# Excalibur-SLE/spmv

Measured on AMD Instinct MI355X. Metric: fp64 CG iters/sec (SpMV effective GB/s vs HBM roofline), higher is better.
Workload: dtype f64

## Files before the change

spmv_amd/csrc/hip/csr_plan.h:

```cpp
#pragma once

#include "common.h"

#include <chrono>
#include <cstdio>

constexpr int kRows = kBlock;

typedef double f64x2 __attribute__((ext_vector_type(2)));
typedef float f32x4 __attribute__((ext_vector_type(4)));
typedef int i32x2 __attribute__((ext_vector_type(2)));
typedef int i32x4 __attribute__((ext_vector_type(4)));

template <typename T>
struct VecOf;
template <>
struct VecOf<double> {
  static constexpr int V = 2;
  using val_t = f64x2;
  using col_t = i32x2;
};
template <>
struct VecOf<float> {
  static constexpr int V = 4;
// ... 81 lines not shown
constexpr int kLxRec = 36;
constexpr int kLxCap = 1344;
constexpr int kLxGap = 16;
constexpr int kLxwPiece = 128;
constexpr int kLxwMaxPieces = 16;
constexpr int kLxwPieces0 = 4;
constexpr int kLxwNpMask = 0xff;
constexpr int kLxwOwnShift = 8;
constexpr int kLxwOwnMask = 0xfffff;
constexpr int kLxwCodedBit = 30;
constexpr int kLxwDict0 = kLxwPieces0 + kLxwMaxPieces;
constexpr int kLxwDictSize = 16;
constexpr int kLxwRec = 28;
__host__ __device__ constexpr int64_t lx_code_bytes(int64_t nnz)
{
  return (((nnz + 1) >> 1) + 16 + 15) & ~(int64_t)15;
}
__host__ __device__ constexpr int64_t lx32_len(int64_t nnz)
{
  return (nnz + 3) & ~(int64_t)3;
}
constexpr int kLxwAlign = 4;
constexpr int kLxwRingValRounds = 2;
constexpr int kLxwRingVcap = kLxwRingValRounds * 1024;
constexpr int kLxwRingCodeMax = 4096;
__host__ __device__ constexpr int lx_ring_code_bytes(int cnt)
{
  return (cnt + 31 + 7) / 8 * 4 + 8;
}
__host__ __device__ constexpr bool lx_ring_fits(int cnt)
{
  return cnt > 0 && cnt + 3 <= kLxwRingVcap
         && lx_ring_code_bytes(cnt) <= kLxwRingCodeMax;
}
constexpr int kXwMaxWin = 8;
constexpr int kXwFirst0 = kLxwPieces0 + kLxwMaxPieces;
constexpr int kXwDelta0 = kXwFirst0 + kXwMaxWin;
constexpr int kXwRec = 36;

constexpr int kLatMaxOff = 8;
constexpr int kLatRec = 12;
constexpr int kWdiaMaxOff = 32;

struct PlanTrace {
  bool on;
  std::chrono::steady_clock::time_point t0;
  const char* who;
  explicit PlanTrace(const char* w)
      : on(getenv("SPMV_PLAN_TRACE") != nullptr), t0(std::chrono::steady_clock::now()),
        who(w)
  {
  }
  void mark(const char* what) const
  {
    if (!on)
      return;
    (void)hipDeviceSynchronize();
    fprintf(stderr, "%s %-14s %9.3f ms\n", who, what,
            std::chrono::duration<double, std::milli>(std::chrono::steady_clock::now()
                                                      - t0)
                .count());
  }
};

template <typename T>
static inline bool aligned16(const T* p)
// ... 136 lines not shown
  int sj_xcd_group = 8;
  struct SpmvTranspose* tr = nullptr;
  void* mv_scratch = nullptr;
  size_t mv_bytes = 0;
  int mv_form = 0;
  int mv_native = 1;
  int32_t* row_list = nullptr;
  int rowlist_exact = 0;
  int32_t num_listed = 0;
  int nt_store = 0;
  int plan_us = 0;
  int plan_mem_us = 0;
  int values_changed_us = 0;
  const int32_t* rowptr0 = nullptr;
  const int32_t* colind0 = nullptr;
  int released = 0;
  int no_new_forms = 0;
  bool structure_baked() const
  {
    return row_list || lx_lidx || lat_tab || slat_mask || t_ptr || lxw_rec
           || xw_rec || wdia_val || sj_lenperm;
  }
  uint16_t* lx_lidx = nullptr;
  int32_t* lx_tab = nullptr;
  int lx = 0;
  int lx_chunks = 2;
  int lx_staged = 0;
  int lx_blocks = 0;
  int32_t* lxw_rec = nullptr;
  int lxw = 0;
  int lxw_max_cnt = 0;
  int lxw_max_pieces = 0;
  int lxw_blocks_per_cu = 0;
  uint8_t* lx_code = nullptr;
  int lx4 = 0;
  int lx4_blocks = 0;
  int lx4_lut = 1;
  int lx_ring_blocks = 0;
  int lx_ring = 1;
  float* lx_val32 = nullptr;
  const void* lx32_values0 = nullptr;
  int lx_v32 = 0;
  int32_t* xw_rec = nullptr;
  int xw = 0;
  int xw_staged = 0;
  int xw_max_cnt = 0, xw_max_pieces = 0;
  struct XwProbe* xw_probe = nullptr;
  int32_t* lat_tab = nullptr;
  uint8_t* lat_mask = nullptr;
  int lat = 0;
  int lat_blocks = 0;
  int lat_blocks_per_cu = 4;
  int lat_xcd_group = 0;
  int lat_chain = 1;

  int lattice_d1 = 0, lattice_d2 = 0;

  int32_t* zw_table = nullptr;
  int zw_slots = 0;
  int zw_grid = 0;
  int zw_segments = 0;
  int64_t zw_d2 = 0;
  int zwalk = 0;

  RowBlockOrder row_block_order(int nrb) const
  {
    RowBlockOrder o;
    o.table = nullptr;
    o.num_slots = 0;
    o.xcd_group = xcd_group;
    o.num_row_blocks = nrb;
// ... 168 lines not shown
```

spmv_amd/csrc/hip/spmv_csr_forms.hip:

```cpp
#include "csr_plan.h"

#include <hipcub/hipcub.hpp>

#include <algorithm>
#include <chrono>
#include <cstring>
#include <new>
#include <utility>
#include <vector>

#include "plan_scratch.h"

namespace
{

template <int ITEMS>
__global__ __launch_bounds__(kBlock) void lx_build_kernel(
    int32_t num_rows, int32_t num_cols, const int32_t* __restrict__ rowptr,
    const int32_t* __restrict__ colind, uint16_t* __restrict__ lidx,
    int32_t* __restrict__ tab, int num_row_blocks, int end_bit, int align,
    int pad, int cap, int32_t* __restrict__ wrec, int32_t* __restrict__ stat,
    int xw)
{
  using Sort = hipcub::BlockRadixSort<int32_t, kBlock, ITEMS, int32_t>;
// ... 174 lines not shown
      }
      s_rank[kLx4Words] = n;
    }
    __syncthreads();
    if (s_rank[kLx4Words] > kLxwDictSize)
      continue;
    for (int w = t; w < kLx4Words; w += kBlock) {
      uint32_t m = s_bits[w];
      int k = s_rank[w];
      while (m) {
        const int b = __ffs(m) - 1;
        m &= m - 1;
        s_dict[k++] = w * 32 + b + kLx4Dmin;
      }
    }
    for (int32_t j = lo; j < hi; ++j) {
      const int b = (int)lidx[j] - t - kLx4Dmin;
      const uint32_t c
          = (uint32_t)(s_rank[b >> 5] + __popc(s_bits[b >> 5] & ((1u << (b & 31)) - 1u)));
      const int q = j - a0;
      atomicOr(&s_pack[q >> 3], c << ((q & 7) * 4));
    }
    __syncthreads();
    for (int w = t; w < nwords; w += kBlock) {
      const bool whole = (w > 0 || a0 == a) && (int64_t)a0 + 8 * (w + 1) <= (int64_t)a + cnt;
      uint32_t* dst = code + ((int64_t)a0 >> 3) + w;
      if (whole)
        *dst = s_pack[w];
      else if (s_pack[w])
        atomicOr(dst, s_pack[w]);
    }
    if (t < kLxwDictSize / 2)
      wr[kLxwDict0 + t] = (s_dict[2 * t] & 0xffff) | (s_dict[2 * t + 1] << 16);
    if (t == 0) {
      wr[3] |= 1 << kLxwCodedBit;
      ++coded;
      ring += lx_ring_fits(cnt) ? 1 : 0;
    }
  }
  if (t == 0 && coded)
    atomicAdd(&stat[0], coded);
  if (t == 0 && ring)
    atomicAdd(&stat[1], ring);
}

struct NonEmptyRow {
  const int32_t* rowptr;
  __device__ bool operator()(int i) const { return rowptr[i + 1] > rowptr[i]; }
};

}

void xw_probe_free(spmv_hip_csr_plan* pl)
{
  if (!pl->xw_probe)
    return;
  for (auto& e : pl->xw_probe->ev)
    for (hipEvent_t& h : e)
      if (h) {
        (void)hipEventDestroy(h);
        h = nullptr;
      }
  delete pl->xw_probe;
  pl->xw_probe = nullptr;
}

void xw_probe_drop_events(XwProbe* pb)
{
  for (auto& e : pb->ev)
    for (hipEvent_t& h : e)
      if (h) {
        (void)hipEventDestroy(h);
        h = nullptr;
      }
}

// ... 37 lines not shown
  hipStream_t st = pl->ctx->stream;
  const int n = pl->num_rows;
  const size_t cap = (size_t)(pl->nnz < n ? pl->nnz : n);
  PlanScratch<int32_t> d_count;
  PlanScratch<void> tmp;
  SPMV_CHECK_HIP(spmv_plan_malloc(&pl->row_list, sizeof(int32_t) * (cap ? cap : 1)));
  hipError_t e = d_count.alloc(1);
  hipcub::CountingInputIterator<int32_t> first(0);
  NonEmptyRow pred{rowptr};
  if (e == hipSuccess)
    e = plan_cub(tmp, [&](void* t, size_t& tb) {
      return hipcub::DeviceSelect::If(t, tb, first, pl->row_list, d_count.get(), n,
                                      pred, st);
    });
  int32_t count = 0;
  if (e == hipSuccess)
    e = plan_fetch(&count, d_count.get(), 1, st);
  tmp.reset();
  d_count.reset();
  if (e != hipSuccess) {
    plan_drop(pl->row_list);
    return static_cast<int>(e);
  }
  pl->num_listed = count;
  return SPMV_HIP_OK;
}

void spmv_free_lx(spmv_hip_csr_plan* pl)
{
  plan_drop(pl->lx_lidx);
  plan_drop(pl->lx_tab);
  plan_drop(pl->lxw_rec);
  plan_drop(pl->lx_code);
  pl->lx = pl->lx_staged = pl->lx_blocks = 0;
  pl->lxw = pl->lxw_max_cnt = pl->lxw_max_pieces = 0;
  pl->lx4 = pl->lx4_blocks = pl->lx_ring_blocks = 0;
  spmv_lx32_free(pl);
}

static int build_lx_codes(spmv_hip_csr_plan* pl, const int32_t* rowptr, int nrb,
                          hipStream_t st)
{
  const size_t bytes = (size_t)lx_code_bytes(pl->nnz);
  PlanScratch<int32_t> d_stat;
  hipError_t e = spmv_plan_malloc(&pl->lx_code, bytes);
  if (e == hipSuccess)
    e = d_stat.alloc(2);
  if (e == hipSuccess)
    e = hipMemsetAsync(pl->lx_code, 0, bytes, st);
  if (e == hipSuccess)
    e = hipMemsetAsync(d_stat.get(), 0, 2 * sizeof(int32_t), st);
  int32_t h_stat[2] = {0, 0};
  if (e == hipSuccess) {
    int grid = pl->ctx->num_cus * 8;
    grid = grid > nrb ? nrb : grid;
    hipLaunchKernelGGL(lx4_encode_kernel, dim3(grid), dim3(kBlock), 0, st,
                       pl->num_rows, rowptr, pl->lx_lidx, pl->lxw_rec,
                       reinterpret_cast<uint32_t*>(pl->lx_code), nrb, d_stat.get());
    e = hipGetLastError();
  }
  if (e == hipSuccess)
    e = plan_fetch(h_stat, d_stat.get(), 2, st);
  d_stat.reset();
  const int32_t coded = h_stat[0];
  if (e != hipSuccess || coded == 0) {
    (void)hipGetLastError();
    plan_drop(pl->lx_code);
    pl->lx4 = pl->lx4_blocks = pl->lx_ring_blocks = 0;
    return e == hipSuccess || e == hipErrorOutOfMemory ? SPMV_HIP_OK
                                                       : static_cast<int>(e);
// ... 321 lines not shown
  PlanScratch<int32_t> d_count;
  PlanScratch<void> tmp;
  int32_t staged = 0;
  if (e == hipSuccess)
    e = d_count.alloc(1);
  hipcub::CountingInputIterator<int32_t> block_ids(0);
  hipcub::TransformInputIterator<int32_t, IsStagedRecord,
                                 hipcub::CountingInputIterator<int32_t>>
      flags(block_ids, IsStagedRecord{pl->lx_tab});
  if (e == hipSuccess)
    e = plan_cub(tmp, [&](void* t, size_t& tb) {
      return hipcub::DeviceReduce::Sum(t, tb, flags, d_count.get(), nrb, st);
    });
  if (e == hipSuccess)
    e = plan_fetch(&staged, d_count.get(), 1, st);
  tmp.reset();
  d_count.reset();
  d_stat.reset();
  if (e != hipSuccess) {
    spmv_free_lx(pl);
    return static_cast<int>(e);
  }
  pl->lx_blocks = nrb;
  pl->lx_staged = staged;
  pl->lxw_max_cnt = h_stat[0];
  pl->lxw_max_pieces = h_stat[1];
  if ((int64_t)staged * 2 < nrb) {
    spmv_free_lx(pl);
    pl->lx_blocks = nrb;
    return SPMV_HIP_OK;
  }
  pl->lx = 1;
  pl->lxw = pl->lxw_rec != nullptr;
  if (pl->lxw_rec && pl->ctx->lx_codes) {
    const int rc = build_lx_codes(pl, rowptr, nrb, st);
    if (rc != SPMV_HIP_OK)
      return rc;
  }
  pl->xcd_group = pl->nontemporal ? 16 : 0;
  {
    const int64_t d2 = spmv_plane_distance(pl, rowptr, colind);
    if (d2 > 0) {
      pl->lattice_d1 = 0;
      pl->lattice_d2 = (int)d2;
      const int rc = spmv_zwalk_order_build(pl, pl->lattice_d2,
                                            spmv_walk_grid(pl), 0, false);
      if (rc != SPMV_HIP_OK)
        return rc;
    }
  }
  return SPMV_HIP_OK;
}

int spmv_walk_grid(const spmv_hip_csr_plan* pl)
{
  if (pl->sdia && pl->sdia_val)
    return spmv_sdia_grid(pl);
  if (pl->symmetric)
    return spmv_slat_grid(pl);
  if (pl->lat_tab)
    return spmv_lat_grid(pl);
  if (pl->lxw && pl->lxw_rec)
    return spmv_lxw_grid(pl, 8);
  return (pl->xw && pl->xw_rec) ? spmv_xw_grid(pl, 8) : spmv_rowblock_grid(pl);
}

// ... 145 lines not shown
```

spmv_amd/csrc/hip/spmv_csr_plan.hip:

```cpp
#include "csr_plan.h"

#include <hipcub/hipcub.hpp>

#include <algorithm>
#include <chrono>
#include <cstring>
#include <new>
#include <utility>
#include <vector>

#include "plan_scratch.h"

thread_local int64_t spmv_plan_mem_ns = 0;

namespace
{
struct MemClock {
  spmv_hip_csr_plan* pl;
  int64_t t0;
  explicit MemClock(spmv_hip_csr_plan* p = nullptr) : pl(p), t0(spmv_plan_mem_ns) {}
  ~MemClock()
  {
    if (pl)
      pl->plan_mem_us += (int)((spmv_plan_mem_ns - t0) / 1000);
// ... 469 lines not shown
    SPMV_REQUIRE(value >= 0 && value <= 4096 && value % 256 == 0);
    plan->sym_window = value;
  } else if (!strcmp(key, "sym_rows")) {
    SPMV_REQUIRE(value == 512 || value == 1024 || value == 2048);
    plan->sym_rows = value;
  } else if (!strcmp(key, "blocks_per_cu")) {
    SPMV_REQUIRE(value >= 1 && value <= kBlocksPerCU);
    plan->blocks_per_cu = value;
    if (plan->zw_table && !plan->lat_tab && !plan->symmetric
        && !plan->sdia_val)
      return spmv_zwalk_order_build(plan, plan->zw_d2, spmv_walk_grid(plan), 0,
                                    true);
  } else if (!strcmp(key, "lx")) {
    SPMV_REQUIRE(value == 0 || plan->lx_lidx);
    plan->lx = value != 0;
  } else if (!strcmp(key, "lxw")) {
    SPMV_REQUIRE(value == 0 || plan->lxw_rec);
    plan->lxw = value != 0;
    if (plan->zw_table && plan->lx_lidx && !plan->lat_tab)
      return spmv_zwalk_order_build(plan, plan->zw_d2, spmv_walk_grid(plan), 0,
                                    true);
  } else if (!strcmp(key, "lx4")) {
    SPMV_REQUIRE(value == 0 || value == 1);
    SPMV_REQUIRE(value == 0 || plan->lx_code);
    plan->lx4 = value;
  } else if (!strcmp(key, "lx_v32")) {
    SPMV_REQUIRE(value == 0 || value == 1);
    SPMV_REQUIRE(value == 0 || plan->lx_val32);
    plan->lx_v32 = value;
  } else if (!strcmp(key, "lx_ring")) {
    SPMV_REQUIRE(value == 0 || value == 1);
    SPMV_REQUIRE(value == 0 || spmv_lxw_ring_ok(plan, true));
    plan->lx_ring = value ? 2 : 0;
  } else if (!strcmp(key, "lx4_lut")) {
    SPMV_REQUIRE(value == 1 || value == 2);
    plan->lx4_lut = value;
  } else if (!strcmp(key, "xw")) {
    SPMV_REQUIRE(value == 0 || plan->xw_rec);
    plan->xw = value != 0;
    if (plan->xw_probe && value) {
      plan->xw_probe->decided = 1;
      plan->xw_probe->use_xw = 1;
    }
    if (plan->zw_table && plan->xw_rec && !plan->lat_tab && !plan->lx_lidx)
      return spmv_zwalk_order_build(plan, plan->zw_d2, spmv_walk_grid(plan), 0,
                                    true);
  } else if (!strcmp(key, "xw_probe")) {
    SPMV_REQUIRE((value == 0 || value == 1) && plan->xw_rec);
    if (!plan->xw_probe)
      plan->xw_probe = new (std::nothrow) XwProbe;
    SPMV_REQUIRE(plan->xw_probe);
    xw_probe_drop_events(plan->xw_probe);
    *plan->xw_probe = XwProbe();
    plan->xw_probe->decided = value ? 0 : 1;
  } else if (!strcmp(key, "lxw_blocks_per_cu")) {
    SPMV_REQUIRE(value >= 0 && value <= kBlocksPerCU);
    plan->lxw_blocks_per_cu = value;
    if (plan->zw_table && !plan->lat_tab
        && ((plan->lxw_rec && plan->lxw) || (plan->xw_rec && plan->xw)))
      return spmv_zwalk_order_build(plan, plan->zw_d2, spmv_walk_grid(plan), 0,
                                    true);
  } else if (!strcmp(key, "lx_chunks")) {
    SPMV_REQUIRE(value == 1 || value == 2);
    plan->lx_chunks = value;
  } else if (!strcmp(key, "nt_store")) {
    plan->nt_store = value != 0;
// ... 221 lines not shown
  else if (!strcmp(key, "xw_pick"))
    *value = !(plan->xw && plan->xw_rec) ? 0
             : !plan->xw_probe           ? 1
             : plan->xw_probe->decided   ? plan->xw_probe->use_xw
                                         : -1;
  else if (!strcmp(key, "xw_probe_xw_us"))
    *value = plan->xw_probe ? (int)plan->xw_probe->us_xw : 0;
  else if (!strcmp(key, "xw_probe_gather_us"))
    *value = plan->xw_probe ? (int)plan->xw_probe->us_gather : 0;
  else if (!strcmp(key, "plan_us"))
    *value = plan->plan_us;
  else if (!strcmp(key, "plan_mem_us"))
    *value = plan->plan_mem_us;
  else if (!strcmp(key, "values_changed_us"))
    *value = plan->values_changed_us;
  else if (!strcmp(key, "mv_form"))
    *value = plan->mv_form;
  else if (!strcmp(key, "mv_native"))
    *value = plan->mv_native;
  else if (!strcmp(key, "mv_kib"))
    *value = (int)((plan->mv_bytes + 1023) / 1024);
  else if (!strcmp(key, "plan_kib")) {
    const int64_t n = plan->num_rows, nnz = plan->nnz;
    const int64_t nrb = (n + kRows - 1) / kRows;
    int64_t b = 0;
    if (plan->row_list)
      b += 4 * (int64_t)plan->num_listed;
    if (plan->lx_lidx)
      b += 2 * (nnz + 8) + 4 * nrb * kLxRec;
    if (plan->lxw_rec)
      b += 4 * nrb * kLxwRec;
    if (plan->lx_code)
      b += lx_code_bytes(nnz);
    if (plan->lx_val32)
      b += 4 * lx32_len(nnz);
    if (plan->xw_rec)
      b += 4 * nrb * kXwRec;
    if (plan->lat_tab)
      b += 48 * nrb + n;
    if (plan->slat_mask)
      b += n;
    const int64_t narr
        = plan->sdia_general == 2 ? 2 * plan->sdia_nd + 1 : plan->sdia_nd + 1;
    if (plan->sdia_val)
      b += narr * plan->sdia_len * plan->sdia_elem + n;
    if (plan->sdia32_val && !plan->sdia_const)
      b += narr * plan->sdia_len * 4 + n;
    if (plan->wdia_val)
      b += (int64_t)plan->wdia_narr * plan->wdia_len * plan->wdia_elem + 4 * n;
    if (plan->wdia32_val && !plan->wdia_const)
      b += (int64_t)plan->wdia_narr * plan->wdia_len * 4;
    if (plan->sj_lenperm)
      b += 4 * ((n + 63) / 64 * 64) + 8 * (int64_t)plan->sj_nblk
           + 4 * (int64_t)plan->sj_nblk * plan->sj_stride
           + (plan->sj_wide_alloc ? 4 : 2) * plan->sj_units * plan->sj_unit
           + 4 * (int64_t)plan->sj_nlong + 4 * ((n + 63) / 64 + 1)
           + 4 * plan->sj_lt_entries + 16 * (int64_t)plan->sj_lt_nsg
           + 2 * plan->sj_lt_codes_n + 8 * (int64_t)plan->sj_nlong;
    if (plan->sj_val)
      b += (int64_t)plan->sj_elem * plan->sj_units * plan->sj_unit;
    if (plan->sj_val32)
      b += 4 * plan->sj_units * plan->sj_unit;
    if (plan->sjt && plan->sjt->sj_lenperm) {
      const spmv_hip_csr_plan* c = plan->sjt;
      b += 4 * (n + 1) + (plan->sjv_map ? 4 * c->nnz : 0);
      if (plan->sj_long_rows)
// ... 50 lines not shown
    *value = plan->zwalk && plan->zw_table ? 1 : 0;
  else if (!strcmp(key, "zwalk_segments"))
    *value = plan->zw_table ? plan->zw_segments : 0;
  else if (!strcmp(key, "zwalk_grid"))
    *value = plan->zw_table ? plan->zw_grid : 0;
  else if (!strcmp(key, "lattice_d1"))
    *value = plan->lattice_d1;
  else if (!strcmp(key, "lattice_d2"))
    *value = plan->lattice_d2;
  else if (!strcmp(key, "lat"))
    *value = plan->lat;
  else if (!strcmp(key, "lat_chain"))
    *value = plan->lat_chain;
  else if (!strcmp(key, "lat_blocks"))
    *value = plan->lat_blocks;
  else if (!strcmp(key, "lx"))
    *value = plan->lx;
  else if (!strcmp(key, "lxw"))
    *value = plan->lxw && plan->lxw_rec ? 1 : 0;
  else if (!strcmp(key, "lx4"))
    *value = plan->lx4 && plan->lx_code ? 1 : 0;
  else if (!strcmp(key, "lx4_blocks"))
    *value = plan->lx_code ? plan->lx4_blocks : 0;
  else if (!strcmp(key, "lx4_all"))
    *value = plan->lx_code && plan->lx4_blocks == plan->lx_staged ? 1 : 0;
  else if (!strcmp(key, "lx4_lut"))
    *value = plan->lx4_lut;
  else if (!strcmp(key, "lx_v32"))
    *value = plan->lx_v32 && plan->lx_val32 ? 1 : 0;
  else if (!strcmp(key, "lx_ring"))
    *value = spmv_lxw_ring_ok(plan, false) ? 1 : 0;
  else if (!strcmp(key, "lx_ring_blocks"))
    *value = plan->lx_code ? plan->lx_ring_blocks : 0;
  else if (!strcmp(key, "lxw_grid"))
    *value = plan->lxw_rec ? spmv_lxw_grid(plan, 8) : 0;
  else if (!strcmp(key, "lx_staged"))
    *value = plan->lx_staged;
  else if (!strcmp(key, "lx_blocks"))
    *value = plan->lx_blocks;
  else if (!strcmp(key, "blocks_per_cu"))
    *value = plan->blocks_per_cu;
  else if (!strcmp(key, "nontemporal"))
    *value = plan->nontemporal;
  else
    return spmv_tr_get(plan, key, value);
  return SPMV_HIP_OK;
}

}
```

spmv_amd/csrc/hip/spmv_lxw.hip:

```cpp
#include "csr_plan.h"
#include "lat_dma.h"

#include <new>
#include <type_traits>

namespace
{

struct LxwBlock {
  int rb;
  int nwin;
  int32_t a;
  int32_t cnt;
  int np;
  int own;
  int coded;
};

template <int REC>
__device__ __forceinline__ int32_t lxw_fetch(int rb,
                                             const int32_t* __restrict__ rec)
{
  int32_t w = 0;
  if (rb >= 0) {
// ... 340 lines not shown
    step(gB, gA);
  }
  if (r_late >= 0)
    out[r_late] = y_late;
  if constexpr (DOT)
    spmv_dot_epilogue(dot, dot_acc, s_red);
}

__device__ __forceinline__ int32_t ring_ld32(const int32_t* p)
{
  int32_t v;
  asm volatile("global_load_dword %0, %1, off" : "=v"(v) : "v"(p) : "memory");
  return v;
}
__device__ __forceinline__ double ring_ld64(const double* p)
{
  double v;
  asm volatile("global_load_dwordx2 %0, %1, off" : "=v"(v) : "v"(p) : "memory");
  return v;
}
__device__ __forceinline__ void ring_st64(double* p, double v)
{
  asm volatile("global_store_dwordx2 %0, %1, off" : : "v"(p), "v"(v) : "memory");
}
template <int N>
__device__ __forceinline__ void ring_wait(int32_t& a, int32_t& b, double& c,
                                          int32_t& d, int32_t& e)
{
  asm volatile("s_waitcnt vmcnt(%5)"
               : "+v"(a), "+v"(b), "+v"(c), "+v"(d), "+v"(e)
               : "n"(N)
               : "memory");
}

template <bool DOT, bool NT, bool TAB, int VR, int PWR>
__global__ __launch_bounds__(kBlock) void csr_lxw_ring_kernel(
    int32_t num_rows, int32_t num_cols, int64_t nnz,
    const int32_t* __restrict__ rowptr, const float* __restrict__ values,
    const uint8_t* __restrict__ code, const int32_t* __restrict__ rec,
    double alpha, const double* __restrict__ in, double beta,
    double* __restrict__ out, DotOut dot, RowBlockOrder ord, int ccap, int xcap)
{
  using T = double;
  constexpr int NW = kBlock / 64;
  constexpr int VCAP = VR * NW * 256;
  constexpr int DMA = VR + 1 + PWR;
  extern __shared__ __attribute__((aligned(16))) unsigned char smem[];
  float* const s_val = reinterpret_cast<float*>(smem);
  unsigned char* const s_code = smem + 3 * (size_t)VCAP * sizeof(float);
  T* const s_x = reinterpret_cast<T*>(s_code + 3 * (size_t)ccap);
  __shared__ double s_red[NW];
  __shared__ int32_t s_dict[3 * kLxwDictSize / 2];
  const unsigned lds_val = (unsigned)(uintptr_t)(
      (__attribute__((address_space(3))) void*)s_val);
  const unsigned lds_code = lds_val + 3u * VCAP * (unsigned)sizeof(float);
  const unsigned lds_x = lds_code + 3u * (unsigned)ccap;
  const unsigned lds_dump = lds_x + 3u * (unsigned)xcap * (unsigned)sizeof(T);

  const int t = threadIdx.x;
  const int wave = __builtin_amdgcn_readfirstlane(t >> 6);
  const int lane = t & 63;
  const int stride = gridDim.x;
  const int num_slots = order_slots(ord);
  double dot_acc = 0.0;
  const int32_t col_last = (num_cols - 2) & ~1;
  const int64_t code_len = lx_code_bytes(nnz);
  const int64_t val_len = lx32_len(nnz);
  const int64_t vdump = lane * 4 < val_len - 4 ? lane * 4 : val_len - 4;
  const int64_t cdump = lane * 16 < code_len - 16 ? lane * 16 : code_len - 16;
  const int32_t xdump = lane * 2 < col_last ? lane * 2 : col_last;

  auto issue = [&](const LxwBlock& b, int32_t w, int sl) {
    const bool live = b.rb >= 0;
    const int64_t a = b.a, e = (int64_t)b.a + b.cnt;
    {
      const int64_t base = a & ~(int64_t)3;
      const int64_t jclamp = (e - 1) & ~(int64_t)3;
      const int pieces = live ? (int)(((e - base) * 4 + 1023) >> 10) : 0;
#pragma unroll
      for (int r = 0; r < VR; ++r) {
        const int q = wave + NW * r;
        const bool real = q < pieces;
        int64_t j = base + (int64_t)(q * 64 + lane) * 4;
        j = j < jclamp ? j : jclamp;
        j = real ? j : vdump;
        glds16<NT>(values + j,
                   real ? lds_val + (unsigned)(sl * VCAP * 4 + q * 1024)
                        : lds_dump);
      }
    }
    {
      const int64_t base = (a >> 1) & ~(int64_t)15, end = (e + 1) >> 1;
      const int64_t jclamp = (end - 1) & ~(int64_t)15;
      const int pieces = live ? (int)((end - base + 1023) >> 10) : 0;
      const bool real = wave < pieces;
      int64_t j = base + (int64_t)(wave * 64 + lane) * 16;
      j = j < jclamp ? j : jclamp;
      j = real ? j : cdump;
      glds16<NT>(code + j, real ? lds_code + (unsigned)(sl * ccap + wave * 1024)
                                : lds_dump);
    }
    const int np = live ? b.np : 0;
#pragma unroll
    for (int k = 0; k < PWR; ++k) {
      const int p = wave + NW * k;
      const bool real = p < np;
      const int32_t col = __builtin_amdgcn_readlane(w, kLxwPieces0 + p);
      int32_t c = col + lane * 2;
      c = c < col_last ? c : col_last;
      c = real ? c : xdump;
      glds16<false>(in + c,
                    real ? lds_x + (unsigned)((sl * xcap + p * kLxwPiece) * 8)
                         : lds_dump);
    }
  };
  auto put_dict = [&](const LxwBlock& b, int32_t w, int sl) {
    if (b.rb >= 0 && t >= kLxwDict0 && t < kLxwDict0 + kLxwDictSize / 2)
      s_dict[sl * (kLxwDictSize / 2) + t - kLxwDict0] = w;
  };
  auto raw_of = [&](int i) {
    if constexpr (TAB)
      return ring_ld32(ord.table + (i < num_slots ? i : num_slots - 1));
    else
      return order_slot_raw_t<false>(ord, i, num_slots);
  };
  auto rb_of = [&](int i, int raw) {
    return i < num_slots ? order_slot_decode(ord, raw) : -1;
  };
  auto fetch = [&](int rb) {
    return ring_ld32(rec + (int64_t)(rb < 0 ? 0 : rb) * kLxwRec
                     + (lane < kLxwRec ? lane : kLxwRec - 1));
  };
  auto loads = [&](int rb, int32_t& lo, int32_t& hi, double& y0) {
    int32_t r = (rb < 0 ? 0 : rb) * kRows + t;
    r = r < num_rows ? r : num_rows - 1;
    lo = ring_ld32(rowptr + r);
    hi = ring_ld32(rowptr + r + 1);
    y0 = ring_ld64(out + (beta != 0.0 ? r : (t < num_rows ? t : num_rows - 1)));
  };

  int it = blockIdx.x;
  int32_t raw0 = raw_of(it), raw1 = raw_of(it + stride);
  int32_t raw2 = raw_of(it + 2 * stride), raw3 = raw_of(it + 3 * stride);
  double dz = 0.0;
  ring_wait<0>(raw0, raw1, dz, raw2, raw3);
  const int rb0 = rb_of(it, raw0), rb1 = rb_of(it + stride, raw1);
  int rb2 = rb_of(it + 2 * stride, raw2);
  int32_t w0 = fetch(rb0), w1 = fetch(rb1), w2 = fetch(rb2);
  int32_t iz = 0;
  ring_wait<0>(w0, w1, dz, w2, iz);
  LxwBlock cur = lxw_decode(rb0, w0);
  LxwBlock nxt = lxw_decode(rb1, w1);
  put_dict(cur, w0, 0);
  put_dict(nxt, w1, 1);
  issue(cur, w0, 0);
  issue(nxt, w1, 1);
  int32_t lo, hi;
  double y0;
  loads(cur.rb, lo, hi, y0);
  ring_wait<0>(lo, hi, y0, iz, iz);
  __syncthreads();
  int s0 = 0, s2 = 2;
  T y_late = T(0);
  int32_t r_late = -1;

  while (it < num_slots) {
    if (r_late >= 0)
      ring_st64(out + r_late, y_late);
    r_late = -1;
    int32_t nlo, nhi;
    double ny0;
    loads(nxt.rb, nlo, nhi, ny0);
    const int rb3 = rb_of(it + 3 * stride, raw3);
    int32_t w3 = fetch(rb3);
    int32_t raw4 = raw_of(it + 4 * stride);
    const LxwBlock blk2 = lxw_decode(rb2, w2);
    put_dict(blk2, w2, s2);
    issue(blk2, w2, s2);

    const int32_t r = cur.rb * kRows + t;
    if (cur.rb >= 0 && r < num_rows) {
      T sum = 0;
      T x_own = T(0);
      int32_t j = lo;
      const float* sv = s_val + (size_t)s0 * VCAP + (cur.a & 3) - cur.a;
      const T* sx = s_x + (size_t)s0 * xcap;
      if constexpr (DOT) {
        if (cur.own >= 0)
          x_own = sx[cur.own + t];
      }
      const uint32_t* sc
          = reinterpret_cast<const uint32_t*>(s_code + (size_t)s0 * ccap);
      const int32_t n0 = cur.a & ~31;
      for (; j < hi; j += 8) {
        const unsigned n = (unsigned)(j - n0);
        const uint32_t c_lo = sc[n >> 3], c_hi = sc[(n >> 3) + 1];
        const uint32_t bits = __builtin_amdgcn_alignbit(c_hi, c_lo, (n & 7) * 4);
        unsigned l[8];
        T v[8], xv[8];
#pragma unroll
        for (int k = 0; k < 8; ++k) {
          const int32_t jj = j + k < hi ? j + k : hi - 1;
          v[k] = (T)sv[jj];
        }
#pragma unroll
        for (int k = 0; k < 8; ++k) {
          const unsigned c = (bits >> (4 * k)) & 15u;
          const int32_t d = reinterpret_cast<const int16_t*>(
              s_dict + s0 * (kLxwDictSize / 2))[c];
          l[k] = j + k < hi ? (unsigned)(t + d) : 0u;
        }
#pragma unroll
        for (int k = 0; k < 8; ++k)
          xv[k] = sx[l[k]];
#pragma unroll
        for (int k = 0; k < 8; ++k)
          if (j + k < hi)
            sum += v[k] * xv[k];
      }
      const T c = alpha * sum;
      T y = c;
      if (beta != T(0))
        y = c + beta * y0;
      y_late = y;
      r_late = r;
      if constexpr (DOT) {
        if (cur.own < 0) {
          x_own = ring_ld64(in + r);
          asm volatile("s_waitcnt vmcnt(0)" : "+v"(x_own) : : "memory");
        }
        dot_acc += (double)x_own * (double)c;
      }
    }
    ring_wait<DMA>(nlo, nhi, ny0, w3, raw4);
    __syncthreads();
    cur = nxt;
    nxt = blk2;
    lo = nlo;
    hi = nhi;
    y0 = ny0;
    rb2 = rb3;
    w2 = w3;
    raw3 = raw4;
    s2 = s0;
    s0 = s0 == 2 ? 0 : s0 + 1;
    it += stride;
  }
  ring_wait<0>(lo, hi, y0, w2, raw3);
  if (r_late >= 0)
    ring_st64(out + r_late, y_late);
  if constexpr (DOT)
    spmv_dot_epilogue(dot, dot_acc, s_red);
}

struct LxwGeom {
  int vcap, lcap, xcap;
  size_t lds;
  int per_cu;
};

LxwGeom lxw_geom(const spmv_hip_csr_plan* pl, int elem_bytes, int idx_bytes)
{
  LxwGeom g;
  const bool xw = idx_bytes == 4;
  const int V = 16 / elem_bytes;
  const int max_cnt = xw ? pl->xw_max_cnt : pl->lxw_max_cnt;
  int64_t vb = ((int64_t)(max_cnt + V) * elem_bytes + 1023) & ~1023ll;
  vb = vb < 1024 ? 1024 : (vb > 32768 ? 32768 : vb);
  g.vcap = (int)(vb / elem_bytes);
  int64_t lb = ((int64_t)(g.vcap + 8) * idx_bytes + 1023) & ~1023ll;
  g.lcap = (int)(lb / idx_bytes);
  int np = xw ? pl->xw_max_pieces : pl->lxw_max_pieces;
  np = np < 1 ? 1 : np;
  g.xcap = np * kLxwPiece;
  g.lds = 2 * (size_t)vb + 2 * (size_t)lb + 2 * (size_t)g.xcap * elem_bytes;
  int per = (int)((160 * 1024 - 1024) / (g.lds + 64));
  per = per < 1 ? 1 : (per > kBlocksPerCU ? kBlocksPerCU : per);
  if (pl->lxw_blocks_per_cu > 0 && pl->lxw_blocks_per_cu < per)
    per = pl->lxw_blocks_per_cu;
  g.per_cu = per;
  return g;
}

int lxw_grid(const spmv_hip_csr_plan* pl, int elem_bytes, int idx_bytes)
{
  const LxwGeom g = lxw_geom(pl, elem_bytes, idx_bytes);
  const int nrb = (pl->num_rows + kRows - 1) / kRows;
  int grid = pl->ctx->num_cus * g.per_cu;
  if (grid > pl->ctx->dot_blocks)
    grid = pl->ctx->dot_blocks;
  if (grid > nrb)
    grid = nrb;
  if (grid < 1)
    grid = 1;
  if (grid >= 8)
    grid -= grid % 8;
  return grid;
}

struct LxwRingGeom {
  int ccap, xcap;
  size_t lds;
  int per_cu;
};

LxwRingGeom lxw_ring_geom(const spmv_hip_csr_plan* pl)
{
  LxwRingGeom g;
  const int max_cnt = pl->lxw_max_cnt < 1 ? 1 : pl->lxw_max_cnt;
  g.ccap = (lx_ring_code_bytes(max_cnt) + 1023) & ~1023;
  int np = pl->lxw_max_pieces;
  np = np < 1 ? 1 : np;
  g.xcap = np * kLxwPiece;
  g.lds = 3 * ((size_t)kLxwRingVcap * sizeof(float) + (size_t)g.ccap
               + (size_t)g.xcap * sizeof(double))
          + 1024;
  g.per_cu = (int)((160 * 1024 - 1024) / (g.lds + 256));
  return g;
}

bool lxw_ring_ok(const spmv_hip_csr_plan* pl, bool forced)
{
  const int nrb = (pl->num_rows + kRows - 1) / kRows;
  if (!(forced || pl->lx_ring) || pl->symmetric || !pl->lx || !pl->lxw
      || !pl->lxw_rec || !pl->lx4 || !pl->lx_code || pl->lx4_lut != 1
      || !pl->lx_v32 || !pl->lx_val32)
    return false;
  if (nrb < 1 || pl->lx_staged != nrb || pl->lx4_blocks != nrb
      || pl->lx_ring_blocks != nrb || !lx_ring_fits(pl->lxw_max_cnt)
      || pl->lxw_max_pieces > kLxwMaxPieces)
    return false;
  if (lxw_ring_geom(pl).per_cu < lxw_geom(pl, 8, 2).per_cu)
    return false;
  constexpr int kMinSteps = 128;
  const int grid = lxw_grid(pl, 8, 2);
  return forced || pl->lx_ring >= 2 || (nrb + grid - 1) / grid >= kMinSteps;
}

template <bool DOT>
int lxw_ring_launch(const spmv_hip_csr_plan* pl, hipStream_t st,
                    const int32_t* rowptr, const float* values, double alpha,
                    const double* in, double beta, double* out, DotOut dot)
{
  constexpr int VR = kLxwRingValRounds, PWR = kLxwMaxPieces / (kBlock / 64);
  const LxwRingGeom g = lxw_ring_geom(pl);
  const int nrb = (pl->num_rows + kRows - 1) / kRows;
  const int grid = lxw_grid(pl, 8, 2);
  RowBlockOrder ord = pl->row_block_order(nrb);
  ord.xcd_group = pl->lat_xcd_group;
  if (pl->zwalk && pl->zw_table && pl->zw_grid == grid) {
    ord.table = pl->zw_table;
    ord.num_slots = pl->zw_slots;
  }
  auto kern
      = ord.table
            ? (pl->nontemporal ? csr_lxw_ring_kernel<DOT, true, true, VR, PWR>
                               : csr_lxw_ring_kernel<DOT, false, true, VR, PWR>)
            : (pl->nontemporal ? csr_lxw_ring_kernel<DOT, true, false, VR, PWR>
                               : csr_lxw_ring_kernel<DOT, false, false, VR, PWR>);
  if (g.lds > 48 * 1024)
    SPMV_CHECK_HIP(hipFuncSetAttribute(
        reinterpret_cast<const void*>(kern),
        hipFuncAttributeMaxDynamicSharedMemorySize, (int)g.lds));
  hipLaunchKernelGGL(kern, dim3(grid), dim3(kBlock), g.lds, st, pl->num_rows,
                     pl->num_cols, pl->nnz, rowptr, values, pl->lx_code,
                     pl->lxw_rec, alpha, in, beta, out, dot, ord, g.ccap, g.xcap);
  SPMV_CHECK_LAUNCH();
  return SPMV_HIP_OK;
}

template <typename TV, typename T, bool DOT, bool XW, int C4>
int lxw_launch_c(const spmv_hip_csr_plan* pl, hipStream_t st,
                 const int32_t* rowptr, const int32_t* colind, const TV* values,
                 T alpha, const T* in, T beta, T* out, DotOut dot)
{
  const LxwGeom g = lxw_geom(pl, (int)sizeof(T), XW ? 4 : 2);
  const int vcap = g.vcap * (int)(sizeof(T) / sizeof(TV));
  const int nrb = (pl->num_rows + kRows - 1) / kRows;
  const int grid = lxw_grid(pl, (int)sizeof(T), XW ? 4 : 2);
  RowBlockOrder ord = pl->row_block_order(nrb);
  ord.xcd_group = pl->lat_xcd_group;
  if (pl->zwalk && pl->zw_table && pl->zw_grid == grid) {
    ord.table = pl->zw_table;
    ord.num_slots = pl->zw_slots;
  }
  auto kern
      = ord.table
            ? (pl->nontemporal ? csr_lxw_kernel<TV, T, DOT, true, true, XW, C4>
                               : csr_lxw_kernel<TV, T, DOT, false, true, XW, C4>)
            : (pl->nontemporal ? csr_lxw_kernel<TV, T, DOT, true, false, XW, C4>
                               : csr_lxw_kernel<TV, T, DOT, false, false, XW, C4>);
  if (g.lds > 48 * 1024)
    SPMV_CHECK_HIP(hipFuncSetAttribute(
        reinterpret_cast<const void*>(kern),
        hipFuncAttributeMaxDynamicSharedMemorySize, (int)g.lds));
  hipLaunchKernelGGL(kern, dim3(grid), dim3(kBlock), g.lds, st, pl->num_rows,
                     pl->num_cols, pl->nnz, rowptr, colind, values,
                     XW ? nullptr : pl->lx_lidx, C4 ? pl->lx_code : nullptr,
                     XW ? pl->xw_rec : pl->lxw_rec, alpha, in, beta, out, dot,
                     ord, vcap, g.lcap, g.xcap);
  SPMV_CHECK_LAUNCH();
  return SPMV_HIP_OK;
}

template <typename TV, typename T, bool DOT, bool XW>
int lxw_launch(const spmv_hip_csr_plan* pl, hipStream_t st,
               const int32_t* rowptr, const int32_t* colind, const TV* values,
               T alpha, const T* in, T beta, T* out, DotOut dot)
{
  if constexpr (!XW && std::is_same<TV, float>::value
                && std::is_same<T, double>::value) {
    if (lxw_ring_ok(pl, false))
      return lxw_ring_launch<DOT>(pl, st, rowptr, values, alpha, in, beta, out,
                                  dot);
  }
  if constexpr (!XW) {
    if (pl->lx4 && pl->lx_code)
      return pl->lx4_lut == 2
                 ? lxw_launch_c<TV, T, DOT, XW, 2>(pl, st, rowptr, colind, values,
                                                   alpha, in, beta, out, dot)
                 : lxw_launch_c<TV, T, DOT, XW, 1>(pl, st, rowptr, colind, values,
                                                   alpha, in, beta, out, dot);
  }
  return lxw_launch_c<TV, T, DOT, XW, 0>(pl, st, rowptr, colind, values, alpha,
                                         in, beta, out, dot);
}

}

int spmv_lxw_grid(const spmv_hip_csr_plan* pl, int elem_bytes)
{
  return lxw_grid(pl, elem_bytes, 2);
}

bool spmv_lxw_ring_ok(const spmv_hip_csr_plan* pl, bool forced)
{
  return lxw_ring_ok(pl, forced);
}

int spmv_xw_grid(const spmv_hip_csr_plan* pl, int elem_bytes)
{
  return lxw_grid(pl, elem_bytes, 4);
}

int spmv_lxw_run_f64(const spmv_hip_csr_plan* pl, hipStream_t st,
                     const int32_t* rowptr, const int32_t* colind,
                     const double* values, double alpha, const double* in,
// ... 51 lines not shown
```

Measured before the change: 326.7.

## Replace ring kernel rowptr loads with packed 16-bit row descriptors staged via LDS DMA

Builds a per-row 16-bit descriptor (start offset within the block plus row length) at plan time. The ring kernel then fetches it as part of the async LDS prefetch on one wave, in place of two per-thread rowptr global loads per block. This cuts per-iteration global traffic and shortens the wait chain. The change also masks dummy-lane DMA issues to a single lane, shrinks the LDS dump area, lets the kernel pick a smaller pieces-per-wave template when max pieces allow, and adds a grid cap knob. In exchange it adds plan memory and a build kernel, and blocks with very long rows are no longer eligible for the ring path.

```diff
diff --git a/spmv_amd/csrc/hip/csr_plan.h b/spmv_amd/csrc/hip/csr_plan.h
--- a/spmv_amd/csrc/hip/csr_plan.h
+++ b/spmv_amd/csrc/hip/csr_plan.h
@@ -137,6 +137,15 @@
 {
   return cnt > 0 && cnt + 3 <= kLxwRingVcap
          && lx_ring_code_bytes(cnt) <= kLxwRingCodeMax;
+}
+constexpr int kLxwDescStartBits = 11;
+constexpr int kLxwDescStartMask = (1 << kLxwDescStartBits) - 1;
+constexpr int kLxwDescMaxLen = (1 << (16 - kLxwDescStartBits)) - 1;
+static_assert(kLxwRingVcap <= kLxwDescStartMask + 1, "a row's start needs more bits");
+constexpr int kLxwDescPad = 1024 - kRows * 2;
+__host__ __device__ constexpr int64_t lx_rowdesc_bytes(int64_t num_row_blocks)
+{
+  return num_row_blocks * (kRows * 2) + kLxwDescPad;
 }
 constexpr int kXwMaxWin = 8;
 constexpr int kXwFirst0 = kLxwPieces0 + kLxwMaxPieces;
@@ -339,11 +348,14 @@
   int lxw_max_cnt = 0;
   int lxw_max_pieces = 0;
   int lxw_blocks_per_cu = 0;
+  int lxw_grid_cap = 0;
   uint8_t* lx_code = nullptr;
   int lx4 = 0;
   int lx4_blocks = 0;
   int lx4_lut = 1;
   int lx_ring_blocks = 0;
+  uint16_t* lx_rowdesc = nullptr;
+  int lx_ring_pwr = 0;
   int lx_ring = 1;
   float* lx_val32 = nullptr;
   const void* lx32_values0 = nullptr;
diff --git a/spmv_amd/csrc/hip/spmv_csr_forms.hip b/spmv_amd/csrc/hip/spmv_csr_forms.hip
--- a/spmv_amd/csrc/hip/spmv_csr_forms.hip
+++ b/spmv_amd/csrc/hip/spmv_csr_forms.hip
@@ -230,16 +230,40 @@
     }
     if (t < kLxwDictSize / 2)
       wr[kLxwDict0 + t] = (s_dict[2 * t] & 0xffff) | (s_dict[2 * t + 1] << 16);
+    const bool ringable
+        = !__syncthreads_or(hi - lo > kLxwDescMaxLen) && lx_ring_fits(cnt);
     if (t == 0) {
       wr[3] |= 1 << kLxwCodedBit;
       ++coded;
-      ring += lx_ring_fits(cnt) ? 1 : 0;
+      ring += ringable ? 1 : 0;
     }
   }
   if (t == 0 && coded)
     atomicAdd(&stat[0], coded);
   if (t == 0 && ring)
     atomicAdd(&stat[1], ring);
+}
+
+__global__ __launch_bounds__(kBlock) void lx_rowdesc_kernel(
+    int32_t num_rows, const int32_t* __restrict__ rowptr,
+    const int32_t* __restrict__ wrec, uint16_t* __restrict__ desc,
+    int num_row_blocks)
+{
+  const int t = threadIdx.x;
+  for (int rb = blockIdx.x; rb < num_row_blocks; rb += gridDim.x) {
+    const int32_t* wr = wrec + (int64_t)rb * kLxwRec;
+    const int32_t a = wr[1], cnt = wr[2];
+    const int32_t r = rb * kRows + t;
+    int32_t lo = 0, hi = 0;
+    if (r < num_rows) {
+      lo = rowptr[r];
+      hi = rowptr[r + 1];
+    }
+    const bool too_long = __syncthreads_or(hi - lo > kLxwDescMaxLen);
+    if (wr[0] >= 0 && lx_ring_fits(cnt) && !too_long && r < num_rows)
+      desc[(int64_t)rb * kRows + t]
+          = (uint16_t)((lo - a) | ((hi - lo) << kLxwDescStartBits));
+  }
 }
 
 struct NonEmptyRow {
@@ -343,10 +367,35 @@
   plan_drop(pl->lx_tab);
   plan_drop(pl->lxw_rec);
   plan_drop(pl->lx_code);
+  plan_drop(pl->lx_rowdesc);
   pl->lx = pl->lx_staged = pl->lx_blocks = 0;
   pl->lxw = pl->lxw_max_cnt = pl->lxw_max_pieces = 0;
   pl->lx4 = pl->lx4_blocks = pl->lx_ring_blocks = 0;
   spmv_lx32_free(pl);
+}
+
+static int build_lx_rowdesc(spmv_hip_csr_plan* pl, const int32_t* rowptr, int nrb,
+                            hipStream_t st)
+{
+  const size_t bytes = (size_t)lx_rowdesc_bytes(nrb);
+  hipError_t e = spmv_plan_malloc(&pl->lx_rowdesc, bytes);
+  if (e == hipSuccess)
+    e = hipMemsetAsync(pl->lx_rowdesc, 0, bytes, st);
+  if (e == hipSuccess) {
+    int grid = pl->ctx->num_cus * 8;
+    grid = grid > nrb ? nrb : grid;
+    hipLaunchKernelGGL(lx_rowdesc_kernel, dim3(grid), dim3(kBlock), 0, st,
+                       pl->num_rows, rowptr, pl->lxw_rec, pl->lx_rowdesc, nrb);
+    e = hipGetLastError();
+  }
+  if (e == hipSuccess)
+    e = hipStreamSynchronize(st);
+  if (e != hipSuccess) {
+    (void)hipGetLastError();
+    plan_drop(pl->lx_rowdesc);
+    return e == hipErrorOutOfMemory ? SPMV_HIP_OK : static_cast<int>(e);
+  }
+  return SPMV_HIP_OK;
 }
 
 static int build_lx_codes(spmv_hip_csr_plan* pl, const int32_t* rowptr, int nrb,
@@ -734,6 +783,11 @@
   }
   pl->lx = 1;
   pl->lxw = pl->lxw_rec != nullptr;
+  if (pl->lxw_rec) {
+    const int rc = build_lx_rowdesc(pl, rowptr, nrb, st);
+    if (rc != SPMV_HIP_OK)
+      return rc;
+  }
   if (pl->lxw_rec && pl->ctx->lx_codes) {
     const int rc = build_lx_codes(pl, rowptr, nrb, st);
     if (rc != SPMV_HIP_OK)
diff --git a/spmv_amd/csrc/hip/spmv_csr_plan.hip b/spmv_amd/csrc/hip/spmv_csr_plan.hip
--- a/spmv_amd/csrc/hip/spmv_csr_plan.hip
+++ b/spmv_amd/csrc/hip/spmv_csr_plan.hip
@@ -525,6 +525,12 @@
     SPMV_REQUIRE(value == 0 || value == 1);
     SPMV_REQUIRE(value == 0 || spmv_lxw_ring_ok(plan, true));
     plan->lx_ring = value ? 2 : 0;
+  } else if (!strcmp(key, "lxw_grid_cap")) {
+    SPMV_REQUIRE(value >= 0);
+    plan->lxw_grid_cap = value;
+  } else if (!strcmp(key, "lx_ring_pwr")) {
+    SPMV_REQUIRE(value == 0 || value == 3 || value == 4);
+    plan->lx_ring_pwr = value == 4 ? 4 : 0;
   } else if (!strcmp(key, "lx4_lut")) {
     SPMV_REQUIRE(value == 1 || value == 2);
     plan->lx4_lut = value;
@@ -812,6 +818,8 @@
       b += 4 * nrb * kLxwRec;
     if (plan->lx_code)
       b += lx_code_bytes(nnz);
+    if (plan->lx_rowdesc)
+      b += lx_rowdesc_bytes(nrb);
     if (plan->lx_val32)
       b += 4 * lx32_len(nnz);
     if (plan->xw_rec)
@@ -928,6 +936,12 @@
     *value = spmv_lxw_ring_ok(plan, false) ? 1 : 0;
   else if (!strcmp(key, "lx_ring_blocks"))
     *value = plan->lx_code ? plan->lx_ring_blocks : 0;
+  else if (!strcmp(key, "lxw_grid_cap"))
+    *value = plan->lxw_grid_cap;
+  else if (!strcmp(key, "lx_ring_pwr"))
+    *value = plan->lx_ring_pwr != 4 && plan->lxw_max_pieces <= 12 ? 3 : 4;
+  else if (!strcmp(key, "lx_rowdesc"))
+    *value = plan->lx_rowdesc ? 1 : 0;
   else if (!strcmp(key, "lxw_grid"))
     *value = plan->lxw_rec ? spmv_lxw_grid(plan, 8) : 0;
   else if (!strcmp(key, "lx_staged"))
diff --git a/spmv_amd/csrc/hip/spmv_lxw.hip b/spmv_amd/csrc/hip/spmv_lxw.hip
--- a/spmv_amd/csrc/hip/spmv_lxw.hip
+++ b/spmv_amd/csrc/hip/spmv_lxw.hip
@@ -396,12 +396,24 @@
                : "n"(N)
                : "memory");
 }
-
+template <int N>
+__device__ __forceinline__ void ring_wait(double& c, int32_t& d, int32_t& e)
+{
+  asm volatile("s_waitcnt vmcnt(%3)"
+               : "+v"(c), "+v"(d), "+v"(e)
+               : "n"(N)
+               : "memory");
+}
+
+constexpr int kRingDescWave = 2;
+constexpr int kRingDumpBytes = 64;
+static_assert(lx_ring_code_bytes(kLxwRingVcap - 3) <= kRingDescWave * 1024,
+              "a fitting block's codes reach the descriptor wave's piece");
 template <bool DOT, bool NT, bool TAB, int VR, int PWR>
 __global__ __launch_bounds__(kBlock) void csr_lxw_ring_kernel(
     int32_t num_rows, int32_t num_cols, int64_t nnz,
-    const int32_t* __restrict__ rowptr, const float* __restrict__ values,
-    const uint8_t* __restrict__ code, const int32_t* __restrict__ rec,
+    const float* __restrict__ values, const uint8_t* __restrict__ code,
+    const uint16_t* __restrict__ desc, const int32_t* __restrict__ rec,
     double alpha, const double* __restrict__ in, double beta,
     double* __restrict__ out, DotOut dot, RowBlockOrder ord, int ccap, int xcap)
 {
@@ -413,13 +425,16 @@
   float* const s_val = reinterpret_cast<float*>(smem);
   unsigned char* const s_code = smem + 3 * (size_t)VCAP * sizeof(float);
   T* const s_x = reinterpret_cast<T*>(s_code + 3 * (size_t)ccap);
+  const uint16_t* const s_desc = reinterpret_cast<const uint16_t*>(
+      reinterpret_cast<unsigned char*>(s_x) + 3 * (size_t)xcap * sizeof(T));
   __shared__ double s_red[NW];
   __shared__ int32_t s_dict[3 * kLxwDictSize / 2];
   const unsigned lds_val = (unsigned)(uintptr_t)(
       (__attribute__((address_space(3))) void*)s_val);
   const unsigned lds_code = lds_val + 3u * VCAP * (unsigned)sizeof(float);
   const unsigned lds_x = lds_code + 3u * (unsigned)ccap;
-  const unsigned lds_dump = lds_x + 3u * (unsigned)xcap * (unsigned)sizeof(T);
+  const unsigned lds_desc = lds_x + 3u * (unsigned)xcap * (unsigned)sizeof(T);
+  const unsigned lds_dump = lds_desc + 3u * (unsigned)(kRows * 2);
 
   const int t = threadIdx.x;
   const int wave = __builtin_amdgcn_readfirstlane(t >> 6);
@@ -448,9 +463,10 @@
         int64_t j = base + (int64_t)(q * 64 + lane) * 4;
         j = j < jclamp ? j : jclamp;
         j = real ? j : vdump;
-        glds16<NT>(values + j,
-                   real ? lds_val + (unsigned)(sl * VCAP * 4 + q * 1024)
-                        : lds_dump);
+        if (lane < (real ? 64 : 1))
+          glds16<NT>(values + j,
+                     real ? lds_val + (unsigned)(sl * VCAP * 4 + q * 1024)
+                          : lds_dump);
       }
     }
     {
@@ -461,8 +477,15 @@
       int64_t j = base + (int64_t)(wave * 64 + lane) * 16;
       j = j < jclamp ? j : jclamp;
       j = real ? j : cdump;
-      glds16<NT>(code + j, real ? lds_code + (unsigned)(sl * ccap + wave * 1024)
-                                : lds_dump);
+      const bool dsc = wave == kRingDescWave;
+      const uint8_t* const src
+          = dsc ? reinterpret_cast<const uint8_t*>(desc)
+                      + (int64_t)(live ? b.rb : 0) * (kRows * 2) + (lane & 31) * 16
+                : code + j;
+      if (lane < (dsc ? 32 : real ? 64 : 1))
+        glds16<NT>(src, dsc ? lds_desc + (unsigned)(sl * (kRows * 2))
+                            : real ? lds_code + (unsigned)(sl * ccap + wave * 1024)
+                                   : lds_dump);
     }
     const int np = live ? b.np : 0;
 #pragma unroll
@@ -473,9 +496,10 @@
       int32_t c = col + lane * 2;
       c = c < col_last ? c : col_last;
       c = real ? c : xdump;
-      glds16<false>(in + c,
-                    real ? lds_x + (unsigned)((sl * xcap + p * kLxwPiece) * 8)
-                         : lds_dump);
+      if (lane < (real ? 64 : 1))
+        glds16<false>(in + c,
+                      real ? lds_x + (unsigned)((sl * xcap + p * kLxwPiece) * 8)
+                           : lds_dump);
     }
   };
   auto put_dict = [&](const LxwBlock& b, int32_t w, int sl) {
@@ -495,11 +519,9 @@
     return ring_ld32(rec + (int64_t)(rb < 0 ? 0 : rb) * kLxwRec
                      + (lane < kLxwRec ? lane : kLxwRec - 1));
   };
-  auto loads = [&](int rb, int32_t& lo, int32_t& hi, double& y0) {
+  auto loads = [&](int rb, double& y0) {
     int32_t r = (rb < 0 ? 0 : rb) * kRows + t;
     r = r < num_rows ? r : num_rows - 1;
-    lo = ring_ld32(rowptr + r);
-    hi = ring_ld32(rowptr + r + 1);
     y0 = ring_ld64(out + (beta != 0.0 ? r : (t < num_rows ? t : num_rows - 1)));
   };
 
@@ -519,10 +541,9 @@
   put_dict(nxt, w1, 1);
   issue(cur, w0, 0);
   issue(nxt, w1, 1);
-  int32_t lo, hi;
   double y0;
-  loads(cur.rb, lo, hi, y0);
-  ring_wait<0>(lo, hi, y0, iz, iz);
+  loads(cur.rb, y0);
+  ring_wait<0>(y0, iz, iz);
   __syncthreads();
   int s0 = 0, s2 = 2;
   T y_late = T(0);
@@ -532,9 +553,8 @@
     if (r_late >= 0)
       ring_st64(out + r_late, y_late);
     r_late = -1;
-    int32_t nlo, nhi;
     double ny0;
-    loads(nxt.rb, nlo, nhi, ny0);
+    loads(nxt.rb, ny0);
     const int rb3 = rb_of(it + 3 * stride, raw3);
     int32_t w3 = fetch(rb3);
     int32_t raw4 = raw_of(it + 4 * stride);
@@ -546,7 +566,9 @@
     if (cur.rb >= 0 && r < num_rows) {
       T sum = 0;
       T x_own = T(0);
-      int32_t j = lo;
+      const int32_t dsc = s_desc[s0 * kRows + t];
+      int32_t j = cur.a + (dsc & kLxwDescStartMask);
+      const int32_t hi = j + (dsc >> kLxwDescStartBits);
       const float* sv = s_val + (size_t)s0 * VCAP + (cur.a & 3) - cur.a;
       const T* sx = s_x + (size_t)s0 * xcap;
       if constexpr (DOT) {
@@ -596,12 +618,10 @@
         dot_acc += (double)x_own * (double)c;
       }
     }
-    ring_wait<DMA>(nlo, nhi, ny0, w3, raw4);
+    ring_wait<DMA>(ny0, w3, raw4);
     __syncthreads();
     cur = nxt;
     nxt = blk2;
-    lo = nlo;
-    hi = nhi;
     y0 = ny0;
     rb2 = rb3;
     w2 = w3;
@@ -610,7 +630,7 @@
     s0 = s0 == 2 ? 0 : s0 + 1;
     it += stride;
   }
-  ring_wait<0>(lo, hi, y0, w2, raw3);
+  ring_wait<0>(y0, w2, raw3);
   if (r_late >= 0)
     ring_st64(out + r_late, y_late);
   if constexpr (DOT)
@@ -655,6 +675,8 @@
     grid = pl->ctx->dot_blocks;
   if (grid > nrb)
     grid = nrb;
+  if (pl->lxw_grid_cap > 0 && grid > pl->lxw_grid_cap)
+    grid = pl->lxw_grid_cap;
   if (grid < 1)
     grid = 1;
   if (grid >= 8)
@@ -677,8 +699,8 @@
   np = np < 1 ? 1 : np;
   g.xcap = np * kLxwPiece;
   g.lds = 3 * ((size_t)kLxwRingVcap * sizeof(float) + (size_t)g.ccap
-               + (size_t)g.xcap * sizeof(double))
-          + 1024;
+               + (size_t)g.xcap * sizeof(double) + kRows * 2)
+          + kRingDumpBytes;
   g.per_cu = (int)((160 * 1024 - 1024) / (g.lds + 256));
   return g;
 }
@@ -688,7 +710,7 @@
   const int nrb = (pl->num_rows + kRows - 1) / kRows;
   if (!(forced || pl->lx_ring) || pl->symmetric || !pl->lx || !pl->lxw
       || !pl->lxw_rec || !pl->lx4 || !pl->lx_code || pl->lx4_lut != 1
-      || !pl->lx_v32 || !pl->lx_val32)
+      || !pl->lx_v32 || !pl->lx_val32 || !pl->lx_rowdesc)
     return false;
   if (nrb < 1 || pl->lx_staged != nrb || pl->lx4_blocks != nrb
       || pl->lx_ring_blocks != nrb || !lx_ring_fits(pl->lxw_max_cnt)
@@ -701,12 +723,12 @@
   return forced || pl->lx_ring >= 2 || (nrb + grid - 1) / grid >= kMinSteps;
 }
 
-template <bool DOT>
-int lxw_ring_launch(const spmv_hip_csr_plan* pl, hipStream_t st,
-                    const int32_t* rowptr, const float* values, double alpha,
-                    const double* in, double beta, double* out, DotOut dot)
-{
-  constexpr int VR = kLxwRingValRounds, PWR = kLxwMaxPieces / (kBlock / 64);
+template <bool DOT, int PWR>
+int lxw_ring_launch_p(const spmv_hip_csr_plan* pl, hipStream_t st,
+                      const float* values, double alpha, const double* in,
+                      double beta, double* out, DotOut dot)
+{
+  constexpr int VR = kLxwRingValRounds;
   const LxwRingGeom g = lxw_ring_geom(pl);
   const int nrb = (pl->num_rows + kRows - 1) / kRows;
   const int grid = lxw_grid(pl, 8, 2);
@@ -727,10 +749,22 @@
         reinterpret_cast<const void*>(kern),
         hipFuncAttributeMaxDynamicSharedMemorySize, (int)g.lds));
   hipLaunchKernelGGL(kern, dim3(grid), dim3(kBlock), g.lds, st, pl->num_rows,
-                     pl->num_cols, pl->nnz, rowptr, values, pl->lx_code,
+                     pl->num_cols, pl->nnz, values, pl->lx_code, pl->lx_rowdesc,
                      pl->lxw_rec, alpha, in, beta, out, dot, ord, g.ccap, g.xcap);
   SPMV_CHECK_LAUNCH();
   return SPMV_HIP_OK;
+}
+
+template <bool DOT>
+int lxw_ring_launch(const spmv_hip_csr_plan* pl, hipStream_t st,
+                    const float* values, double alpha, const double* in,
+                    double beta, double* out, DotOut dot)
+{
+  constexpr int NW = kBlock / 64, PWR = kLxwMaxPieces / NW;
+  if (pl->lx_ring_pwr != PWR && pl->lxw_max_pieces <= (PWR - 1) * NW)
+    return lxw_ring_launch_p<DOT, PWR - 1>(pl, st, values, alpha, in, beta, out,
+                                           dot);
+  return lxw_ring_launch_p<DOT, PWR>(pl, st, values, alpha, in, beta, out, dot);
 }
 
 template <typename TV, typename T, bool DOT, bool XW, int C4>
@@ -775,8 +809,7 @@
   if constexpr (!XW && std::is_same<TV, float>::value
                 && std::is_same<T, double>::value) {
     if (lxw_ring_ok(pl, false))
-      return lxw_ring_launch<DOT>(pl, st, rowptr, values, alpha, in, beta, out,
-                                  dot);
+      return lxw_ring_launch<DOT>(pl, st, values, alpha, in, beta, out, dot);
   }
   if constexpr (!XW) {
     if (pl->lx4 && pl->lx_code)
```

Result: faster. 336.0, median of 6 (+2.8%).
